# amathislab/myochallenge

Hardware: AMD Instinct MI355X
Metric: env-steps/sec (Baoding, 4096 envs) (higher is better)
Workload: dtype f64

## Files before the change

myochallenge_amd/csrc/myo_ppo_mlp.h:

```cpp
#pragma once
#ifndef MYO_EMU

typedef __attribute__((ext_vector_type(8))) __bf16 myo_bf16x8;
typedef __attribute__((ext_vector_type(4))) float myo_f32x4;

#define MLP_H 256
#define MLP_OPMAX 128
#define MLP_APM 48
#define MLP_AKP 64
#define MLP_XS (MLP_OPMAX + 8)
#define MLP_HS (MLP_H + 8)
#define MLP_DS (MLP_AKP + 8)
#define MLP_SOS 49
#define MLP_SPLITK 16

struct MlpArgs {
  const float *obs, *act, *oldlp, *adv, *ret;
  const long long* idx;
  const float *log_std, *adv_stats;
  const unsigned short *W1p, *W2, *W2T, *Whp, *WhT;
  const float* bias;
  unsigned short *XT, *H1T, *H2T, *dH1T, *dH2T, *dOT;
  float* part;
  int B, O, A, OP, NB;
// ... 79 lines not shown
  constexpr int PER = 4;
  float v[PER];
  float s = 0.f;
#pragma unroll
  for (int k = 0; k < PER; ++k) { const int i = lo + t + 256 * k; v[k] = i < hi ? adv[idx[i]] : 0.f; s += v[k]; }
  for (int i = lo + t + 256 * PER; i < hi; i += 256) s += adv[idx[i]];
  for (int off = 32; off >= 1; off >>= 1) s += __shfl_xor(s, off, 64);
  if ((t & 63) == 0) red[t >> 6] = s;
  __syncthreads();
  if (t == 0) s_mean = n ? ((red[0] + red[1]) + (red[2] + red[3])) / n : 0.f;
  __syncthreads();
  const float mean = s_mean;
  float m2 = 0.f;
#pragma unroll
  for (int k = 0; k < PER; ++k) { const float d = v[k] - mean; m2 += (lo + t + 256 * k) < hi ? d * d : 0.f; }
  for (int i = lo + t + 256 * PER; i < hi; i += 256) { const float d = adv[idx[i]] - mean; m2 += d * d; }
  for (int off = 32; off >= 1; off >>= 1) m2 += __shfl_xor(m2, off, 64);
  __syncthreads();
  if ((t & 63) == 0) red[t >> 6] = m2;
  __syncthreads();
  if (t == 0) { part[3 * blockIdx.x] = (float)n; part[3 * blockIdx.x + 1] = mean; part[3 * blockIdx.x + 2] = (red[0] + red[1]) + (red[2] + red[3]); }
}

template <int KSTEPS>
__device__ __forceinline__ void mlp_load_w(myo_bf16x8 (&bw)[8][4], const unsigned short* Wg, int w_stride, int n0, int lm, int lq) {
#pragma unroll
  for (int ks = 0; ks < KSTEPS; ++ks)
#pragma unroll
    for (int nt = 0; nt < 4; ++nt) bw[ks][nt] = *reinterpret_cast<const myo_bf16x8*>(Wg + (size_t)(n0 + 16 * nt + lm) * w_stride + 32 * ks + 8 * lq);
  __builtin_amdgcn_sched_barrier(0);
}
template <int KSTEPS, int MT>
__device__ __forceinline__ void mlp_mma_slab(myo_f32x4 (&acc)[MT][4], const unsigned short* As, int as_stride, const myo_bf16x8 (&bw)[8][4],
                                             int lm, int lq) {
#pragma unroll
  for (int mt = 0; mt < MT; ++mt)
#pragma unroll
    for (int nt = 0; nt < 4; ++nt) acc[mt][nt] = myo_f32x4{0.f, 0.f, 0.f, 0.f};
#pragma unroll
  for (int ks = 0; ks < KSTEPS; ++ks) {
#pragma unroll
    for (int m2 = 0; m2 < MT; m2 += 2) {
      myo_bf16x8 a[2];
#pragma unroll
      for (int mt = 0; mt < 2; ++mt) a[mt] = *reinterpret_cast<const myo_bf16x8*>(As + (16 * (m2 + mt) + lm) * as_stride + 32 * ks + 8 * lq);
#pragma unroll
      for (int mt = 0; mt < 2; ++mt)
#pragma unroll
        for (int nt = 0; nt < 4; ++nt) acc[m2 + mt][nt] = __builtin_amdgcn_mfma_f32_16x16x32_bf16(a[mt], bw[ks][nt], acc[m2 + mt][nt], 0, 0, 0);
    }
  }
  __builtin_amdgcn_sched_barrier(0);
}

#ifdef MLP_PROF
__device__ unsigned long long g_mlp_prof[16];
#define MLP_STAMP(k) { __syncthreads(); if (threadIdx.x == 0 && blockIdx.x == 3 && blockIdx.y == 0) g_mlp_prof[k] = wall_clock64(); }
extern "C" int myo_debug_mlp_prof(unsigned long long* out) { return (int)hipMemcpyFromSymbol(out, HIP_SYMBOL(g_mlp_prof), sizeof g_mlp_prof); }
#else
#define MLP_STAMP(k)
#endif

#ifndef MLP_BM
#define MLP_BM 32
#endif
#define MLP_FWDBWD_LDS (512 + MLP_BM * MLP_XS * 2 + MLP_BM * MLP_HS * 2 + MLP_BM * MLP_SOS * 4 + MLP_BM * MLP_DS * 2 + 128 * 4 + 192 * 4)

template <int MT>
__device__ __forceinline__ unsigned long long mlp_store_act(const myo_f32x4 (&acc)[MT][4], const float (&bb)[4], unsigned short* Hs, unsigned short* HT,
                                                            size_t B, int r0, int n0, int lm, int lq) {
  static_assert(MT * 16 <= 64, "one mask bit per accumulator element");
  unsigned long long mask = 0;
#pragma unroll
  for (int mt = 0; mt < MT; ++mt)
#pragma unroll
    for (int nt = 0; nt < 4; ++nt) {
      const int n = n0 + 16 * nt + lm, m = 16 * mt + 4 * lq;
      unsigned short h[4];
#pragma unroll
      for (int r = 0; r < 4; ++r) {
        h[r] = mlp_f2bf(fmaxf(acc[mt][nt][r] + bb[nt], 0.f)); Hs[(m + r) * MLP_HS + n] = h[r];
        mask |= (unsigned long long)(h[r] != 0) << (16 * mt + 4 * nt + r);
      }
      *reinterpret_cast<uint2*>(HT + (size_t)n * B + r0 + m) = make_uint2((unsigned)h[0] | ((unsigned)h[1] << 16), (unsigned)h[2] | ((unsigned)h[3] << 16));
    }
  return mask;
}
template <int MT, bool TO_LDS>
__device__ __forceinline__ void mlp_store_grad(const myo_f32x4 (&acc)[MT][4], unsigned long long mask, unsigned short* Hs, unsigned short* HT, size_t B,
                                               int r0, int n0, int lm, int lq) {
#pragma unroll
  for (int mt = 0; mt < MT; ++mt)
#pragma unroll
    for (int nt = 0; nt < 4; ++nt) {
      const int n = n0 + 16 * nt + lm, m = 16 * mt + 4 * lq;
      unsigned short h[4];
#pragma unroll
      for (int r = 0; r < 4; ++r) {
        const unsigned short on = (unsigned short)(-(int)((mask >> (16 * mt + 4 * nt + r)) & 1ull));
        h[r] = mlp_f2bf(acc[mt][nt][r]) & on;
        if (TO_LDS) Hs[(m + r) * MLP_HS + n] = h[r];
      }
      *reinterpret_cast<uint2*>(HT + (size_t)n * B + r0 + m) = make_uint2((unsigned)h[0] | ((unsigned)h[1] << 16), (unsigned)h[2] | ((unsigned)h[3] << 16));
    }
}

__global__ void __launch_bounds__(256, 2) k_mlp_fwdbwd(MlpArgs P) {
  constexpr int H = MLP_H, XS = MLP_XS, HS = MLP_HS, DS = MLP_DS, SOS = MLP_SOS, BM = MLP_BM, MT = BM / 16, RW = BM / 4;
  extern __shared__ __align__(16) unsigned char mlp_smem[];
  long long* s_idx = reinterpret_cast<long long*>(mlp_smem);
  unsigned short* Xs = reinterpret_cast<unsigned short*>(mlp_smem + 512);
  float* So = reinterpret_cast<float*>(mlp_smem + 512);
  unsigned short* Hs = Xs + BM * XS;
  float* Sa = reinterpret_cast<float*>(Hs + BM * HS);
  unsigned short* dOs = reinterpret_cast<unsigned short*>(Sa + BM * SOS);
  float* s_ls = reinterpret_cast<float*>(dOs + BM * DS);
  float* s_row = s_ls + 128;
  static_assert(BM * MLP_SOS * 4 <= BM * MLP_XS * 2, "the head output tile fits where X was");
  static_assert(BM == 32 || BM == 64, "wave / tile mapping below");
  const int t = threadIdx.x, w = t >> 6, lane = t & 63, lm = lane & 15, lq = lane >> 4;
  const int net = blockIdx.y, blk = blockIdx.x, r0 = blk * BM, B = P.B, O = P.O, A = P.A, OP = P.OP;
  const int n0 = 64 * w;
  MLP_STAMP(0)
  if (t < BM) s_idx[t] = P.idx[r0 + t];
  if (t < A) { const float ls = P.log_std[t]; s_ls[t] = ls; s_ls[64 + t] = __expf(-ls); }
  const float* b1 = P.bias + net * H; const float* b2 = P.bias + 2 * H + net * H; const float* bh = P.bias + 4 * H + net * MLP_APM;
  float bb1[4], bb2[4];
#pragma unroll
  for (int nt = 0; nt < 4; ++nt) { bb1[nt] = b1[n0 + 16 * nt + lm]; bb2[nt] = b2[n0 + 16 * nt + lm]; }
  myo_bf16x8 bw[8][4];
  {
    const unsigned short* W1 = P.W1p + (size_t)net * H * OP;
    if (OP == 96) mlp_load_w<3>(bw, W1, OP, n0, lm, lq);
    else if (OP == 128) mlp_load_w<4>(bw, W1, OP, n0, lm, lq);
    else if (OP == 64) mlp_load_w<2>(bw, W1, OP, n0, lm, lq);
    else mlp_load_w<1>(bw, W1, OP, n0, lm, lq);
  }
  __syncthreads();
  if (t < BM) {
    const size_t src = (size_t)s_idx[t];
    s_row[t] = P.adv[src]; s_row[64 + t] = P.oldlp[src]; s_row[128 + t] = P.ret[src];
  }
  {
    float v[RW][2], av[RW];
#pragma unroll
    for (int k = 0; k < RW; ++k) {
      const size_t row = (size_t)s_idx[RW * w + k];
      v[k][0] = lane < O ? P.obs[row * O + lane] : 0.f;
      v[k][1] = lane + 64 < O ? P.obs[row * O + lane + 64] : 0.f;
      av[k] = (net == 0 && lane < A) ? P.act[row * A + lane] : 0.f;
    }
#pragma unroll
    for (int k = 0; k < RW; ++k) {
      Xs[(RW * w + k) * XS + lane] = mlp_f2bf(v[k][0]);
      if (lane + 64 < OP) Xs[(RW * w + k) * XS + lane + 64] = mlp_f2bf(v[k][1]);
      if (lane < A) Sa[(RW * w + k) * SOS + lane] = av[k];
    }
    if (net == 0) {
#pragma unroll
      for (int h = 0; h < 2; ++h) {
        const int c = lane + 64 * h;
        if (c < OP) {
          unsigned u[RW / 2];
#pragma unroll
          for (int k = 0; k < RW / 2; ++k) u[k] = (unsigned)mlp_f2bf(v[2 * k][h]) | ((unsigned)mlp_f2bf(v[2 * k + 1][h]) << 16);
          uint4* dst = reinterpret_cast<uint4*>(P.XT + (size_t)c * B + r0 + RW * w);
#pragma unroll
          for (int q = 0; q < RW / 8; ++q) dst[q] = make_uint4(u[4 * q], u[4 * q + 1], u[4 * q + 2], u[4 * q + 3]);
        }
      }
    }
  }
  __syncthreads();
  MLP_STAMP(1)
  myo_f32x4 acc[MT][4];
  if (OP == 96) mlp_mma_slab<3, MT>(acc, Xs, XS, bw, lm, lq);
  else if (OP == 128) mlp_mma_slab<4, MT>(acc, Xs, XS, bw, lm, lq);
  else if (OP == 64) mlp_mma_slab<2, MT>(acc, Xs, XS, bw, lm, lq);
  else mlp_mma_slab<1, MT>(acc, Xs, XS, bw, lm, lq);
  mlp_load_w<H / 32>(bw, P.W2 + (size_t)net * H * H, H, n0, lm, lq);
  const unsigned long long mask1 = mlp_store_act<MT>(acc, bb1, Hs, P.H1T + (size_t)net * H * B, B, r0, n0, lm, lq);
  __syncthreads();
  MLP_STAMP(2)
  mlp_mma_slab<H / 32, MT>(acc, Hs, HS, bw, lm, lq);
  const unsigned short* Wh = P.Whp + (size_t)net * MLP_APM * H;
  myo_bf16x8 bh2[H / 32];
  if (w < 3) {
#pragma unroll
    for (int ks = 0; ks < H / 32; ++ks) bh2[ks] = *reinterpret_cast<const myo_bf16x8*>(Wh + (size_t)(16 * w + lm) * H + 32 * ks + 8 * lq);
  }
  __builtin_amdgcn_sched_barrier(0);
  __syncthreads();
  const unsigned long long mask2 = mlp_store_act<MT>(acc, bb2, Hs, P.H2T + (size_t)net * H * B, B, r0, n0, lm, lq);
  __syncthreads();
  MLP_STAMP(3)
  if (w < 3) {
    const float bv = bh[16 * w + lm];
#pragma unroll
    for (int mt = 0; mt < MT; ++mt) {
      myo_f32x4 ah = myo_f32x4{0.f, 0.f, 0.f, 0.f};
#pragma unroll
      for (int ks = 0; ks < H / 32; ++ks) {
        const myo_bf16x8 a = *reinterpret_cast<const myo_bf16x8*>(Hs + (16 * mt + lm) * HS + 32 * ks + 8 * lq);
        ah = __builtin_amdgcn_mfma_f32_16x16x32_bf16(a, bh2[ks], ah, 0, 0, 0);
      }
#pragma unroll
      for (int r = 0; r < 4; ++r) So[(16 * mt + 4 * lq + r) * SOS + 16 * w + lm] = ah[r] + bv;
    }
  }
  mlp_load_w<MLP_AKP / 32>(bw, P.WhT + (size_t)net * H * MLP_AKP, MLP_AKP, n0, lm, lq);
  __syncthreads();
  MLP_STAMP(4)
  const int NB = P.NB;
  if (w == 0) {
    const int r = lane < BM ? lane : 0;
    const bool on = lane < BM;
    if (net == 0) {
      float logp = 0.f;
      for (int a = 0; a < A; ++a) {
        const float z = (Sa[r * SOS + a] - So[r * SOS + a]) * s_ls[64 + a];
        logp += -0.5f * z * z - s_ls[a] - 0.9189385332046727f;
      }
      const float an = (s_row[r] - P.adv_stats[0]) / (P.adv_stats[1] + 1e-8f);
      const float clip = P.hp ? P.hp[MYO_HP_CLIP] : P.clip;
      const float lr_i = logp - s_row[64 + r];
      const float ratio = __expf(lr_i);
      const float s1 = an * ratio;
      const float rc = fminf(fmaxf(ratio, 1.f - clip), 1.f + clip);
      const float s2 = an * rc;
      float pl_i = on ? -fminf(s1, s2) / B : 0.f;
      const bool inside = (ratio > 1.f - clip) && (ratio < 1.f + clip);
      const float dlogp = -(an * ratio) * ((s1 <= s2) ? 1.f : (inside ? 1.f : 0.f)) / B;
      if (on) {
        for (int a = 0; a < A; ++a) {
          const float inv = s_ls[64 + a];
          const float z = (Sa[r * SOS + a] - So[r * SOS + a]) * inv;
          const float dm = dlogp * z * inv;
          So[r * SOS + a] = dm;
          Sa[r * SOS + a] = dlogp * (z * z - 1.f);
          dOs[r * DS + a] = mlp_f2bf(dm);
        }
        for (int a = A; a < MLP_AKP; ++a) dOs[r * DS + a] = 0;
      }
      for (int off = 32; off >= 1; off >>= 1) pl_i += __shfl_xor(pl_i, off, 64);
      if (lane == 0) P.part[(size_t)A * NB + blk] = pl_i;
      if (P.hp) {
        float ent = 0.f;
        for (int a = 0; a < A; ++a) ent += s_ls[a] + 1.4189385332046727f;
        float kl_i = on ? ((ratio - 1.f) - lr_i) / B : 0.f, cf_i = on ? (fabsf(ratio - 1.f) > clip ? 1.f : 0.f) / B : 0.f;
        float el_i = on ? -ent / B : 0.f;
        for (int off = 32; off >= 1; off >>= 1) {
          kl_i += __shfl_xor(kl_i, off, 64); cf_i += __shfl_xor(cf_i, off, 64); el_i += __shfl_xor(el_i, off, 64);
        }
        if (lane == 0) {
          P.part[(size_t)(2 * A + 3) * NB + blk] = kl_i; P.part[(size_t)(2 * A + 4) * NB + blk] = cf_i;
          P.part[(size_t)(2 * A + 5) * NB + blk] = el_i;
        }
      }
    } else {
      const float dv = So[r * SOS] - s_row[128 + r];
      float vl_i = on ? dv * dv / B : 0.f, dv_i = on ? P.vf_coef * 2.f / B * dv : 0.f;
      if (on) {
        dOs[r * DS] = mlp_f2bf(dv_i);
        for (int a = 1; a < MLP_AKP; ++a) dOs[r * DS + a] = 0;
      }
      for (int off = 32; off >= 1; off >>= 1) { vl_i += __shfl_xor(vl_i, off, 64); dv_i += __shfl_xor(dv_i, off, 64); }
      if (lane == 0) { P.part[(size_t)(A + 1) * NB + blk] = vl_i; P.part[(size_t)(2 * A + 2) * NB + blk] = dv_i; }
    }
  }
  __syncthreads();
  MLP_STAMP(5)
  if (net == 0 && t < A) {
    float my_ls = 0.f, my_db = 0.f;
    for (int r = 0; r < BM; ++r) { my_ls += Sa[r * SOS + t]; my_db += So[r * SOS + t]; }
    P.part[(size_t)t * NB + blk] = my_ls; P.part[(size_t)(A + 2 + t) * NB + blk] = my_db;
  }
  {
    const int Ah = net == 0 ? A : 1;
    for (int e = t; e < Ah * (BM / 8); e += 256) {
      const int c = e / (BM / 8), ch = e % (BM / 8);
      unsigned v[4];
#pragma unroll
      for (int k = 0; k < 4; ++k) v[k] = (unsigned)dOs[(8 * ch + 2 * k) * DS + c] | ((unsigned)dOs[(8 * ch + 2 * k + 1) * DS + c] << 16);
      *reinterpret_cast<uint4*>(P.dOT + ((size_t)net * 128 + c) * B + r0 + 8 * ch) = make_uint4(v[0], v[1], v[2], v[3]);
    }
  }
  MLP_STAMP(6)
  mlp_mma_slab<MLP_AKP / 32, MT>(acc, dOs, DS, bw, lm, lq);
  mlp_load_w<H / 32>(bw, P.W2T + (size_t)net * H * H, H, n0, lm, lq);
  mlp_store_grad<MT, true>(acc, mask2, Hs, P.dH2T + (size_t)net * H * B, B, r0, n0, lm, lq);
  __syncthreads();
  MLP_STAMP(7)
  mlp_mma_slab<H / 32, MT>(acc, Hs, HS, bw, lm, lq);
  mlp_store_grad<MT, false>(acc, mask1, Hs, P.dH1T + (size_t)net * H * B, B, r0, n0, lm, lq);
  MLP_STAMP(8)
}

struct MlpPolicyArgs {
  const float* obs;
  const float* log_std;
  const unsigned short *W1p, *W2, *Whp;
  const float* bias;
  float* obs_buf;
  float *act_buf, *val_buf, *logp_buf, *clipped;
  const int* t_idx;
  unsigned long long* draw_counter;
  unsigned long long seed;
  int N, O, A, OP, deterministic;
};
#define MLP_POLICY_LDS (MLP_BM * MLP_XS * 2 + MLP_BM * MLP_HS * 2 + 128 * 4)

template <int MT>
__device__ __forceinline__ void mlp_store_act_lds(const myo_f32x4 (&acc)[MT][4], const float (&bb)[4], unsigned short* Hs, int n0, int lm, int lq) {
#pragma unroll
  for (int mt = 0; mt < MT; ++mt)
#pragma unroll
    for (int nt = 0; nt < 4; ++nt) {
      const int n = n0 + 16 * nt + lm, m = 16 * mt + 4 * lq;
#pragma unroll
      for (int r = 0; r < 4; ++r) Hs[(m + r) * MLP_HS + n] = mlp_f2bf(fmaxf(acc[mt][nt][r] + bb[nt], 0.f));
    }
}

__global__ void __launch_bounds__(256, 2) k_mlp_policy(MlpPolicyArgs P) {
  constexpr int H = MLP_H, XS = MLP_XS, HS = MLP_HS, SOS = MLP_SOS, BM = MLP_BM, MT = BM / 16, RW = BM / 4;
  extern __shared__ __align__(16) unsigned char mlp_smem[];
  unsigned short* Xs = reinterpret_cast<unsigned short*>(mlp_smem);
  float* So = reinterpret_cast<float*>(mlp_smem);
  unsigned short* Hs = Xs + BM * XS;
  float* s_ls = reinterpret_cast<float*>(Hs + BM * HS);
  static_assert(BM * MLP_SOS * 4 <= BM * MLP_XS * 2, "the head output tile fits where X was");
  const int t = threadIdx.x, w = t >> 6, lane = t & 63, lm = lane & 15, lq = lane >> 4;
  const int net = blockIdx.y, r0 = blockIdx.x * BM, N = P.N, O = P.O, A = P.A, OP = P.OP;
  const int n0 = 64 * w;
  const size_t tt = (size_t)(*P.t_idx);
  if (t < A) { const float ls = P.log_std[t]; s_ls[t] = ls; s_ls[64 + t] = __expf(ls); }
  const float* b1 = P.bias + net * H; const float* b2 = P.bias + 2 * H + net * H; const float* bh = P.bias + 4 * H + net * MLP_APM;
  float bb1[4], bb2[4];
#pragma unroll
  for (int nt = 0; nt < 4; ++nt) { bb1[nt] = b1[n0 + 16 * nt + lm]; bb2[nt] = b2[n0 + 16 * nt + lm]; }
  myo_bf16x8 bw[8][4];
  {
    const unsigned short* W1 = P.W1p + (size_t)net * H * OP;
    if (OP == 96) mlp_load_w<3>(bw, W1, OP, n0, lm, lq);
    else if (OP == 128) mlp_load_w<4>(bw, W1, OP, n0, lm, lq);
    else if (OP == 64) mlp_load_w<2>(bw, W1, OP, n0, lm, lq);
    else mlp_load_w<1>(bw, W1, OP, n0, lm, lq);
  }
  {
    float v[RW][2];
#pragma unroll
    for (int k = 0; k < RW; ++k) {
      const size_t row = (size_t)(r0 + RW * w + k);
      v[k][0] = lane < O ? P.obs[row * O + lane] : 0.f;
      v[k][1] = lane + 64 < O ? P.obs[row * O + lane + 64] : 0.f;
    }
#pragma unroll
    for (int k = 0; k < RW; ++k) {
      Xs[(RW * w + k) * XS + lane] = mlp_f2bf(v[k][0]);
      if (lane + 64 < OP) Xs[(RW * w + k) * XS + lane + 64] = mlp_f2bf(v[k][1]);
      if (net == 0 && P.obs_buf) {
        float* dst = P.obs_buf + (tt * N + (size_t)(r0 + RW * w + k)) * O;
        if (lane < O) dst[lane] = v[k][0];
        if (lane + 64 < O) dst[lane + 64] = v[k][1];
      }
    }
  }
  __syncthreads();
  myo_f32x4 acc[MT][4];
  if (OP == 96) mlp_mma_slab<3, MT>(acc, Xs, XS, bw, lm, lq);
  else if (OP == 128) mlp_mma_slab<4, MT>(acc, Xs, XS, bw, lm, lq);
  else if (OP == 64) mlp_mma_slab<2, MT>(acc, Xs, XS, bw, lm, lq);
  else mlp_mma_slab<1, MT>(acc, Xs, XS, bw, lm, lq);
  mlp_load_w<H / 32>(bw, P.W2 + (size_t)net * H * H, H, n0, lm, lq);
  mlp_store_act_lds<MT>(acc, bb1, Hs, n0, lm, lq);
  __syncthreads();
  mlp_mma_slab<H / 32, MT>(acc, Hs, HS, bw, lm, lq);
  const unsigned short* Wh = P.Whp + (size_t)net * MLP_APM * H;
  myo_bf16x8 bh2[H / 32];
  if (w < 3) {
#pragma unroll
    for (int ks = 0; ks < H / 32; ++ks) bh2[ks] = *reinterpret_cast<const myo_bf16x8*>(Wh + (size_t)(16 * w + lm) * H + 32 * ks + 8 * lq);
  }
  __builtin_amdgcn_sched_barrier(0);
  __syncthreads();
  mlp_store_act_lds<MT>(acc, bb2, Hs, n0, lm, lq);
  __syncthreads();
  if (w < 3) {
    const float bv = bh[16 * w + lm];
#pragma unroll
    for (int mt = 0; mt < MT; ++mt) {
      myo_f32x4 ah = myo_f32x4{0.f, 0.f, 0.f, 0.f};
#pragma unroll
      for (int ks = 0; ks < H / 32; ++ks) {
        const myo_bf16x8 a = *reinterpret_cast<const myo_bf16x8*>(Hs + (16 * mt + lm) * HS + 32 * ks + 8 * lq);
        ah = __builtin_amdgcn_mfma_f32_16x16x32_bf16(a, bh2[ks], ah, 0, 0, 0);
      }
#pragma unroll
      for (int r = 0; r < 4; ++r) So[(16 * mt + 4 * lq + r) * SOS + 16 * w + lm] = ah[r] + bv;
    }
  }
  __syncthreads();
  if (net == 1) {
    if (t < BM) P.val_buf[tt * N + r0 + t] = So[t * SOS];
    return;
  }
  const unsigned long long ctr = P.draw_counter[0];
  const int row = t >> 3, g0 = t & 7, i = r0 + row;
  float logp = 0.f;
  static_assert(BM * 8 == 256, "8 lanes per row");
  for (int a0 = 4 * g0; a0 < A; a0 += 32) {
    unsigned int c[4] = {(unsigned int)i, (unsigned int)(a0 >> 2), (unsigned int)ctr, (unsigned int)(ctr >> 32)};
    unsigned int k0 = (unsigned int)P.seed, k1 = (unsigned int)(P.seed >> 32);
    for (int r = 0; r < 10; ++r) { philox_round(c, k0, k1); k0 += 0x9E3779B9u; k1 += 0xBB67AE85u; }
    float z[4];
    for (int h = 0; h < 2; ++h) {
      const float u1 = ((float)(c[2 * h] >> 8) + 0.5f) * (1.0f / 16777216.0f);
      const float u2 = ((float)(c[2 * h + 1] >> 8) + 0.5f) * (1.0f / 16777216.0f);
      const float rad = sqrtf(-2.0f * __logf(u1));
      float sn, cs;
      __sincosf(6.283185307179586f * u2, &sn, &cs);
      z[2 * h] = rad * cs; z[2 * h + 1] = rad * sn;
    }
#pragma unroll
    for (int k = 0; k < 4; ++k) {
      const int a = a0 + k;
      if (a < A) {
        const float mu = So[row * SOS + a], ls = s_ls[a];
        const float act = P.deterministic ? mu : mu + s_ls[64 + a] * z[k];
        const float zz = (act - mu) * __expf(-ls);
        logp += -0.5f * zz * zz - ls - 0.9189385332046727f;
        P.act_buf[(tt * N + i) * A + a] = act;
        P.clipped[(size_t)i * A + a] = fminf(fmaxf(act, -1.f), 1.f);
// ... 143 lines not shown
```

myochallenge_amd/csrc/myobatch.hip:

```cpp
#include <hip/hip_runtime.h>
#include <utility>
#include <vector>
#define MYO_BACKEND_NAME "gfx950"
#define MYO_BACKEND_DENSE_NEWTON 0
#define MYO_BACKEND_BATCH_FIELDS hipEvent_t ev0, ev1; std::vector<std::pair<hipEvent_t, hipEvent_t>> pending;
#include "myo_host.h"

typedef hipStream_t be_stream;
static int be_malloc(void** p, size_t n) { return (int)hipMalloc(p, n ? n : 1); }
static void be_free(void* p) { (void)hipFree(p); }
static int be_h2d(void* d, const void* h, size_t n) { return (int)hipMemcpy(d, h, n, hipMemcpyHostToDevice); }
static int be_set_device(int dev) { return (int)hipSetDevice(dev); }
static const char* be_errstr(int e) { return hipGetErrorString((hipError_t)e); }

#define MYO_MAX_DEVICES 64
struct BoundDev { const myo_batch* b = nullptr; hipStream_t last = nullptr; bool have_last = false; hipEvent_t ev = nullptr; };
static BoundDev g_bound[MYO_MAX_DEVICES];
static std::mutex g_bound_mu;
struct SlotWs { double* p = nullptr; int* map = nullptr; int users = 0; char* big = nullptr; int big_users = 0; };
static SlotWs g_slot_ws[MYO_MAX_DEVICES];
static bool slot_workspace_acquire(int device, double** ws, int** map) {
  if (device < 0 || device >= MYO_MAX_DEVICES) return false;
  std::lock_guard<std::mutex> lk(g_bound_mu);
  SlotWs& w = g_slot_ws[device];
// ... 1793 lines not shown
  hipStream_t st = (hipStream_t)stream;
  static bool lds_set = false;
  if (!lds_set) {
    if (hipFuncSetAttribute((const void*)k_mlp_fwdbwd, hipFuncAttributeMaxDynamicSharedMemorySize, MLP_FWDBWD_LDS) != hipSuccess)
      return fail(MYO_E_DEVICE, "myo_ppo_mlp_step: cannot reserve %d bytes of LDS", (int)MLP_FWDBWD_LDS);
    lds_set = true;
  }
  if (d->compute_adv_stats) hipLaunchKernelGGL(k_adv_moments, dim3(MLP_ADV_BLOCKS), dim3(256), 0, st, d->adv, (const long long*)d->idx, B, w.advpart);
  MlpPrepArgs pp;
  pp.p = d->params; pp.O = O; pp.OP = OP; pp.Ah[0] = A; pp.Ah[1] = 1;
  for (int k = 0; k < 2; ++k) {
    pp.off_W1[k] = d->off_W1[k]; pp.off_b1[k] = d->off_b1[k]; pp.off_W2[k] = d->off_W2[k]; pp.off_b2[k] = d->off_b2[k];
    pp.off_Wh[k] = d->off_Wh[k]; pp.off_bh[k] = d->off_bh[k];
  }
  pp.adv_part = w.advpart; pp.adv_stats = d->adv_stats; pp.adv_nb = d->compute_adv_stats ? MLP_ADV_BLOCKS : 0; pp.B = B;
  pp.W1p = w.W1p; pp.W2 = w.W2; pp.W2T = w.W2T; pp.Whp = w.Whp; pp.WhT = w.WhT; pp.bias = w.bias;
  hipLaunchKernelGGL(k_mlp_prep, dim3(256), dim3(256), 0, st, pp);
  MlpArgs a;
  a.obs = d->obs; a.act = d->act; a.oldlp = d->oldlp; a.adv = d->adv; a.ret = d->ret; a.idx = (const long long*)d->idx;
  a.log_std = d->params + d->off_log_std; a.adv_stats = d->adv_stats;
  a.W1p = w.W1p; a.W2 = w.W2; a.W2T = w.W2T; a.Whp = w.Whp; a.WhT = w.WhT; a.bias = w.bias;
  a.XT = w.XT; a.H1T = w.H1T; a.H2T = w.H2T; a.dH1T = w.dH1T; a.dH2T = w.dH2T; a.dOT = w.dOT; a.part = w.part;
  a.B = B; a.O = O; a.A = A; a.OP = OP; a.NB = B / MLP_BM; a.clip = d->clip; a.vf_coef = d->vf_coef; a.hp = d->hp;
  hipLaunchKernelGGL(k_mlp_fwdbwd, dim3(B / MLP_BM, 2), dim3(256), MLP_FWDBWD_LDS, st, a);
  MlpWgradArgs g;
  g.njobs = 0; g.B = B; g.rows_per_split = B / MLP_SPLITK; g.G = d->G; g.slab = w.slab;
  const size_t HB = (size_t)MLP_H * B;
  for (int net = 0; net < 2; ++net) {
    for (int m0 = 0; m0 < MLP_H; m0 += 128) {
      for (int n0 = 0; n0 < MLP_H; n0 += 128)
        g.job[g.njobs++] = MlpWgradJob{w.dH2T + net * HB, w.H1T + net * HB, MLP_H, MLP_H, MLP_H, m0, n0, d->off_W2[net], n0 == 0 ? d->off_b2[net] : -1};
      g.job[g.njobs++] = MlpWgradJob{w.dH1T + net * HB, w.XT, MLP_H, O, O, m0, 0, d->off_W1[net], d->off_b1[net]};
    }
    for (int n0 = 0; n0 < MLP_H; n0 += 128)
      g.job[g.njobs++] = MlpWgradJob{w.dOT + (size_t)net * 128 * B, w.H2T + net * HB, net == 0 ? A : 1, MLP_H, MLP_H, 0, n0, d->off_Wh[net], -1};
  }
  hipLaunchKernelGGL(k_mlp_wgrad, dim3(g.njobs * MLP_SPLITK), dim3(256), 0, st, g);
  if (d->sqnorm_part && d->adam_step) {
    MlpRfArgs rf;
    rf.slab = w.slab; rf.g = d->grads; rf.G = d->G; rf.splits = MLP_SPLITK; rf.part = w.part; rf.acc = d->acc; rf.NB = B / MLP_BM; rf.A = A;
    rf.ent_coef = d->ent_coef; rf.off_log_std = d->off_log_std; rf.off_bh0 = d->off_bh[0]; rf.off_bh1 = d->off_bh[1];
    rf.sq_part = d->sqnorm_part; rf.adam_step = d->adam_step; rf.hp = d->hp;
    hipLaunchKernelGGL(k_mlp_reduce_finish, dim3(MLP_RF_BLOCKS + 2 * A + 3), dim3(256), 0, st, rf);
  } else {
    hipLaunchKernelGGL(k_mlp_reduce, dim3((unsigned)((d->G + 255) / 256)), dim3(256), 0, st, (const float*)w.slab, d->grads, d->G, MLP_SPLITK);
    hipLaunchKernelGGL(k_colmajor_finish, dim3(2 * A + 3 + (d->hp ? 1 : 0)), dim3(64), 0, st, (const float*)w.part, d->acc, B / MLP_BM, A, d->ent_coef,
                       d->grads + d->off_log_std, d->grads + d->off_bh[0], d->grads + d->off_bh[1], d->hp);
// ... 31 lines not shown
  pp.p = d->params; pp.O = d->O; pp.OP = OP; pp.Ah[0] = d->A; pp.Ah[1] = 1;
  for (int k = 0; k < 2; ++k) {
    pp.off_W1[k] = d->off_W1[k]; pp.off_b1[k] = d->off_b1[k]; pp.off_W2[k] = d->off_W2[k]; pp.off_b2[k] = d->off_b2[k];
    pp.off_Wh[k] = d->off_Wh[k]; pp.off_bh[k] = d->off_bh[k];
  }
  pp.adv_part = nullptr; pp.adv_stats = nullptr; pp.adv_nb = 0; pp.B = 0;
  pp.W1p = w.W1p; pp.W2 = w.W2; pp.W2T = w.W2T; pp.Whp = w.Whp; pp.WhT = w.WhT; pp.bias = w.bias;
  hipLaunchKernelGGL(k_mlp_prep, dim3(256), dim3(256), 0, (hipStream_t)stream, pp);
  LAUNCH_CHECK(0)
  return MYO_OK;
}
extern "C" int myo_ppo_mlp_rollout(const myo_ppo_mlp_rollout_desc* d, void* stream) {
  if (!d || !d->obs || !d->params || !d->draw_counter || !d->t_idx || !d->act_buf || !d->val_buf || !d->logp_buf || !d->clipped || !d->workspace)
    return fail(MYO_E_ARG, "myo_ppo_mlp_rollout: null argument");
  if (!mlp_rollout_ok(d)) return fail(MYO_E_UNSUPPORTED, "myo_ppo_mlp_rollout: needs hidden = %d, obs <= %d, act <= %d, envs a multiple of %d", MLP_H, MLP_OPMAX, MLP_APM, MLP_BM);
  const int OP = (d->O + 31) / 32 * 32;
  const MlpImg w = mlp_carve_images((unsigned char*)d->workspace, OP);
  if ((long long)w.bytes > d->workspace_bytes) return fail(MYO_E_ARG, "myo_ppo_mlp_rollout: workspace too small (%zu bytes needed)", w.bytes);
  MlpPolicyArgs a;
  a.obs = d->obs; a.log_std = d->params + d->off_log_std; a.W1p = w.W1p; a.W2 = w.W2; a.Whp = w.Whp; a.bias = w.bias;
  a.obs_buf = d->obs_buf; a.act_buf = d->act_buf; a.val_buf = d->val_buf; a.logp_buf = d->logp_buf; a.clipped = d->clipped;
  a.t_idx = d->t_idx; a.draw_counter = (unsigned long long*)d->draw_counter; a.seed = d->seed;
  a.N = d->N; a.O = d->O; a.A = d->A; a.OP = OP; a.deterministic = d->deterministic;
  hipLaunchKernelGGL(k_mlp_policy, dim3(d->N / MLP_BM, 2), dim3(256), MLP_POLICY_LDS, (hipStream_t)stream, a);
  LAUNCH_CHECK(0)
  return MYO_OK;
}

#include "myo_lstm_step.h"
extern "C" int myo_lstm_step_supported(int H) { return (H == 32 || H == 64 || H == 128 || H == 256) ? 1 : 0; }
extern "C" int myo_lstm_step_fwd(const void* gx, long long gx_sg, long long gx_sr, const void* h_prev, const void* c_prev, const void* w_hh,
                                 const float* keep_next, int G, int N, int H, void* out_h, long long out_sg, void* hm_next, void* cm_next,
                                 void* c_new, void* ws, const float* c_prev32, float* cm_next32, void* stream) {
  if (!gx || !h_prev || (!c_prev && !c_prev32) || !w_hh || !out_h || !hm_next || (!cm_next && !cm_next32) || G <= 0 || N <= 0 || H <= 0 || (gx_sg & 3) || (gx_sr & 3) || (out_sg & 3))
    return fail(MYO_E_ARG, "myo_lstm_step_fwd: bad arguments");
  if (!myo_lstm_step_supported(H)) return fail(MYO_E_UNSUPPORTED, "myo_lstm_step_fwd: hidden size %d (32, 64, 128 or 256)", H);
  typedef const unsigned short* cu;
  typedef unsigned short* mu;
#define MYO_LSTM_FWD(HH)                                                                                                              \
  lstm_step_fwd_launch<HH>((cu)gx, gx_sg, gx_sr, (cu)h_prev, (cu)c_prev, (cu)w_hh, keep_next, G, N, (mu)out_h, out_sg, (mu)hm_next,   \
                           (mu)cm_next, (mu)c_new, (mu)ws, c_prev32, cm_next32, (hipStream_t)stream)
  switch (H) {
    case 32: MYO_LSTM_FWD(32); break;
    case 64: MYO_LSTM_FWD(64); break;
    case 128: MYO_LSTM_FWD(128); break;
    default: MYO_LSTM_FWD(256); break;
  }
// ... 61 lines not shown
```

Before: 1.727 million.

## Split MLP kernels across eight waves and parallelize the log-prob epilogue

Widens the fused PPO MLP forward/backward and policy kernels from 4 to 8 waves per block, so each wave owns 32 hidden columns instead of 64. This halves the per-wave weight-register and accumulator footprint and raises occupancy per block. The serial single-wave log-prob and gradient epilogue is redistributed so every wave handles its own rows, one action column per lane, with an extra LDS staging tile and additional barriers. The trade-off is more block-wide synchronisation, and in the policy kernel half the threads leave early during the sampling tail.

Result: no change. 1.739 million (median of 6 runs) (+0.7%).

```diff
diff --git a/myochallenge_amd/csrc/myo_ppo_mlp.h b/myochallenge_amd/csrc/myo_ppo_mlp.h
--- a/myochallenge_amd/csrc/myo_ppo_mlp.h
+++ b/myochallenge_amd/csrc/myo_ppo_mlp.h
@@ -125,21 +125,24 @@
   if (t == 0) { part[3 * blockIdx.x] = (float)n; part[3 * blockIdx.x + 1] = mean; part[3 * blockIdx.x + 2] = (red[0] + red[1]) + (red[2] + red[3]); }
 }
 
-template <int KSTEPS>
-__device__ __forceinline__ void mlp_load_w(myo_bf16x8 (&bw)[8][4], const unsigned short* Wg, int w_stride, int n0, int lm, int lq) {
+#define MLP_WAVES 8
+#define MLP_NT (MLP_H / 16 / MLP_WAVES)
+#define MLP_THREADS (64 * MLP_WAVES)
+template <int KSTEPS, int NT>
+__device__ __forceinline__ void mlp_load_w(myo_bf16x8 (&bw)[8][NT], const unsigned short* Wg, int w_stride, int n0, int lm, int lq) {
 #pragma unroll
   for (int ks = 0; ks < KSTEPS; ++ks)
 #pragma unroll
-    for (int nt = 0; nt < 4; ++nt) bw[ks][nt] = *reinterpret_cast<const myo_bf16x8*>(Wg + (size_t)(n0 + 16 * nt + lm) * w_stride + 32 * ks + 8 * lq);
+    for (int nt = 0; nt < NT; ++nt) bw[ks][nt] = *reinterpret_cast<const myo_bf16x8*>(Wg + (size_t)(n0 + 16 * nt + lm) * w_stride + 32 * ks + 8 * lq);
   __builtin_amdgcn_sched_barrier(0);
 }
-template <int KSTEPS, int MT>
-__device__ __forceinline__ void mlp_mma_slab(myo_f32x4 (&acc)[MT][4], const unsigned short* As, int as_stride, const myo_bf16x8 (&bw)[8][4],
+template <int KSTEPS, int MT, int NT>
+__device__ __forceinline__ void mlp_mma_slab(myo_f32x4 (&acc)[MT][NT], const unsigned short* As, int as_stride, const myo_bf16x8 (&bw)[8][NT],
                                              int lm, int lq) {
 #pragma unroll
   for (int mt = 0; mt < MT; ++mt)
 #pragma unroll
-    for (int nt = 0; nt < 4; ++nt) acc[mt][nt] = myo_f32x4{0.f, 0.f, 0.f, 0.f};
+    for (int nt = 0; nt < NT; ++nt) acc[mt][nt] = myo_f32x4{0.f, 0.f, 0.f, 0.f};
 #pragma unroll
   for (int ks = 0; ks < KSTEPS; ++ks) {
 #pragma unroll
@@ -150,7 +153,7 @@
 #pragma unroll
       for (int mt = 0; mt < 2; ++mt)
 #pragma unroll
-        for (int nt = 0; nt < 4; ++nt) acc[m2 + mt][nt] = __builtin_amdgcn_mfma_f32_16x16x32_bf16(a[mt], bw[ks][nt], acc[m2 + mt][nt], 0, 0, 0);
+        for (int nt = 0; nt < NT; ++nt) acc[m2 + mt][nt] = __builtin_amdgcn_mfma_f32_16x16x32_bf16(a[mt], bw[ks][nt], acc[m2 + mt][nt], 0, 0, 0);
     }
   }
   __builtin_amdgcn_sched_barrier(0);
@@ -169,38 +172,38 @@
 #endif
 #define MLP_FWDBWD_LDS (512 + MLP_BM * MLP_XS * 2 + MLP_BM * MLP_HS * 2 + MLP_BM * MLP_SOS * 4 + MLP_BM * MLP_DS * 2 + 128 * 4 + 192 * 4)
 
-template <int MT>
-__device__ __forceinline__ unsigned long long mlp_store_act(const myo_f32x4 (&acc)[MT][4], const float (&bb)[4], unsigned short* Hs, unsigned short* HT,
-                                                            size_t B, int r0, int n0, int lm, int lq) {
-  static_assert(MT * 16 <= 64, "one mask bit per accumulator element");
-  unsigned long long mask = 0;
+template <int MT, int NT>
+__device__ __forceinline__ unsigned mlp_store_act(const myo_f32x4 (&acc)[MT][NT], const float (&bb)[NT], unsigned short* Hs, unsigned short* HT,
+                                                  size_t B, int r0, int n0, int lm, int lq) {
+  static_assert(MT * NT * 4 <= 32, "one mask bit per accumulator element");
+  unsigned mask = 0;
 #pragma unroll
   for (int mt = 0; mt < MT; ++mt)
 #pragma unroll
-    for (int nt = 0; nt < 4; ++nt) {
+    for (int nt = 0; nt < NT; ++nt) {
       const int n = n0 + 16 * nt + lm, m = 16 * mt + 4 * lq;
       unsigned short h[4];
 #pragma unroll
       for (int r = 0; r < 4; ++r) {
         h[r] = mlp_f2bf(fmaxf(acc[mt][nt][r] + bb[nt], 0.f)); Hs[(m + r) * MLP_HS + n] = h[r];
-        mask |= (unsigned long long)(h[r] != 0) << (16 * mt + 4 * nt + r);
+        mask |= (unsigned)(h[r] != 0) << (4 * NT * mt + 4 * nt + r);
       }
       *reinterpret_cast<uint2*>(HT + (size_t)n * B + r0 + m) = make_uint2((unsigned)h[0] | ((unsigned)h[1] << 16), (unsigned)h[2] | ((unsigned)h[3] << 16));
     }
   return mask;
 }
-template <int MT, bool TO_LDS>
-__device__ __forceinline__ void mlp_store_grad(const myo_f32x4 (&acc)[MT][4], unsigned long long mask, unsigned short* Hs, unsigned short* HT, size_t B,
+template <int MT, int NT, bool TO_LDS>
+__device__ __forceinline__ void mlp_store_grad(const myo_f32x4 (&acc)[MT][NT], unsigned mask, unsigned short* Hs, unsigned short* HT, size_t B,
                                                int r0, int n0, int lm, int lq) {
 #pragma unroll
   for (int mt = 0; mt < MT; ++mt)
 #pragma unroll
-    for (int nt = 0; nt < 4; ++nt) {
+    for (int nt = 0; nt < NT; ++nt) {
       const int n = n0 + 16 * nt + lm, m = 16 * mt + 4 * lq;
       unsigned short h[4];
 #pragma unroll
       for (int r = 0; r < 4; ++r) {
-        const unsigned short on = (unsigned short)(-(int)((mask >> (16 * mt + 4 * nt + r)) & 1ull));
+        const unsigned short on = (unsigned short)(-(int)((mask >> (4 * NT * mt + 4 * nt + r)) & 1u));
         h[r] = mlp_f2bf(acc[mt][nt][r]) & on;
         if (TO_LDS) Hs[(m + r) * MLP_HS + n] = h[r];
       }
@@ -208,36 +211,39 @@
     }
 }
 
-__global__ void __launch_bounds__(256, 2) k_mlp_fwdbwd(MlpArgs P) {
-  constexpr int H = MLP_H, XS = MLP_XS, HS = MLP_HS, DS = MLP_DS, SOS = MLP_SOS, BM = MLP_BM, MT = BM / 16, RW = BM / 4;
+__global__ void __launch_bounds__(MLP_THREADS, 4) k_mlp_fwdbwd(MlpArgs P) {
+  constexpr int H = MLP_H, XS = MLP_XS, HS = MLP_HS, DS = MLP_DS, SOS = MLP_SOS, BM = MLP_BM, MT = BM / 16, NT = MLP_NT, NW = MLP_WAVES, RW = BM / NW;
   extern __shared__ __align__(16) unsigned char mlp_smem[];
   long long* s_idx = reinterpret_cast<long long*>(mlp_smem);
   unsigned short* Xs = reinterpret_cast<unsigned short*>(mlp_smem + 512);
   float* So = reinterpret_cast<float*>(mlp_smem + 512);
   unsigned short* Hs = Xs + BM * XS;
+  float* St = reinterpret_cast<float*>(Hs);
   float* Sa = reinterpret_cast<float*>(Hs + BM * HS);
   unsigned short* dOs = reinterpret_cast<unsigned short*>(Sa + BM * SOS);
   float* s_ls = reinterpret_cast<float*>(dOs + BM * DS);
   float* s_row = s_ls + 128;
   static_assert(BM * MLP_SOS * 4 <= BM * MLP_XS * 2, "the head output tile fits where X was");
+  static_assert(BM * MLP_SOS * 4 <= BM * MLP_HS * 2, "the log-prob terms fit where H2 was");
   static_assert(BM == 32 || BM == 64, "wave / tile mapping below");
+  static_assert(NT * 16 * NW == H && (RW == 4 || RW == 8), "wave / column mapping below");
   const int t = threadIdx.x, w = t >> 6, lane = t & 63, lm = lane & 15, lq = lane >> 4;
   const int net = blockIdx.y, blk = blockIdx.x, r0 = blk * BM, B = P.B, O = P.O, A = P.A, OP = P.OP;
-  const int n0 = 64 * w;
+  const int n0 = 16 * NT * w;
   MLP_STAMP(0)
   if (t < BM) s_idx[t] = P.idx[r0 + t];
   if (t < A) { const float ls = P.log_std[t]; s_ls[t] = ls; s_ls[64 + t] = __expf(-ls); }
   const float* b1 = P.bias + net * H; const float* b2 = P.bias + 2 * H + net * H; const float* bh = P.bias + 4 * H + net * MLP_APM;
-  float bb1[4], bb2[4];
-#pragma unroll
-  for (int nt = 0; nt < 4; ++nt) { bb1[nt] = b1[n0 + 16 * nt + lm]; bb2[nt] = b2[n0 + 16 * nt + lm]; }
-  myo_bf16x8 bw[8][4];
+  float bb1[NT], bb2[NT];
+#pragma unroll
+  for (int nt = 0; nt < NT; ++nt) { bb1[nt] = b1[n0 + 16 * nt + lm]; bb2[nt] = b2[n0 + 16 * nt + lm]; }
+  myo_bf16x8 bw[8][NT];
   {
     const unsigned short* W1 = P.W1p + (size_t)net * H * OP;
-    if (OP == 96) mlp_load_w<3>(bw, W1, OP, n0, lm, lq);
-    else if (OP == 128) mlp_load_w<4>(bw, W1, OP, n0, lm, lq);
-    else if (OP == 64) mlp_load_w<2>(bw, W1, OP, n0, lm, lq);
-    else mlp_load_w<1>(bw, W1, OP, n0, lm, lq);
+    if (OP == 96) mlp_load_w<3, NT>(bw, W1, OP, n0, lm, lq);
+    else if (OP == 128) mlp_load_w<4, NT>(bw, W1, OP, n0, lm, lq);
+    else if (OP == 64) mlp_load_w<2, NT>(bw, W1, OP, n0, lm, lq);
+    else mlp_load_w<1, NT>(bw, W1, OP, n0, lm, lq);
   }
   __syncthreads();
   if (t < BM) {
@@ -267,25 +273,25 @@
           unsigned u[RW / 2];
 #pragma unroll
           for (int k = 0; k < RW / 2; ++k) u[k] = (unsigned)mlp_f2bf(v[2 * k][h]) | ((unsigned)mlp_f2bf(v[2 * k + 1][h]) << 16);
-          uint4* dst = reinterpret_cast<uint4*>(P.XT + (size_t)c * B + r0 + RW * w);
-#pragma unroll
-          for (int q = 0; q < RW / 8; ++q) dst[q] = make_uint4(u[4 * q], u[4 * q + 1], u[4 * q + 2], u[4 * q + 3]);
+          uint2* dst = reinterpret_cast<uint2*>(P.XT + (size_t)c * B + r0 + RW * w);
+#pragma unroll
+          for (int q = 0; q < RW / 4; ++q) dst[q] = make_uint2(u[2 * q], u[2 * q + 1]);
         }
       }
     }
   }
   __syncthreads();
   MLP_STAMP(1)
-  myo_f32x4 acc[MT][4];
-  if (OP == 96) mlp_mma_slab<3, MT>(acc, Xs, XS, bw, lm, lq);
-  else if (OP == 128) mlp_mma_slab<4, MT>(acc, Xs, XS, bw, lm, lq);
-  else if (OP == 64) mlp_mma_slab<2, MT>(acc, Xs, XS, bw, lm, lq);
-  else mlp_mma_slab<1, MT>(acc, Xs, XS, bw, lm, lq);
-  mlp_load_w<H / 32>(bw, P.W2 + (size_t)net * H * H, H, n0, lm, lq);
-  const unsigned long long mask1 = mlp_store_act<MT>(acc, bb1, Hs, P.H1T + (size_t)net * H * B, B, r0, n0, lm, lq);
+  myo_f32x4 acc[MT][NT];
+  if (OP == 96) mlp_mma_slab<3, MT, NT>(acc, Xs, XS, bw, lm, lq);
+  else if (OP == 128) mlp_mma_slab<4, MT, NT>(acc, Xs, XS, bw, lm, lq);
+  else if (OP == 64) mlp_mma_slab<2, MT, NT>(acc, Xs, XS, bw, lm, lq);
+  else mlp_mma_slab<1, MT, NT>(acc, Xs, XS, bw, lm, lq);
+  mlp_load_w<H / 32, NT>(bw, P.W2 + (size_t)net * H * H, H, n0, lm, lq);
+  const unsigned mask1 = mlp_store_act<MT, NT>(acc, bb1, Hs, P.H1T + (size_t)net * H * B, B, r0, n0, lm, lq);
   __syncthreads();
   MLP_STAMP(2)
-  mlp_mma_slab<H / 32, MT>(acc, Hs, HS, bw, lm, lq);
+  mlp_mma_slab<H / 32, MT, NT>(acc, Hs, HS, bw, lm, lq);
   const unsigned short* Wh = P.Whp + (size_t)net * MLP_APM * H;
   myo_bf16x8 bh2[H / 32];
   if (w < 3) {
@@ -294,7 +300,7 @@
   }
   __builtin_amdgcn_sched_barrier(0);
   __syncthreads();
-  const unsigned long long mask2 = mlp_store_act<MT>(acc, bb2, Hs, P.H2T + (size_t)net * H * B, B, r0, n0, lm, lq);
+  const unsigned mask2 = mlp_store_act<MT, NT>(acc, bb2, Hs, P.H2T + (size_t)net * H * B, B, r0, n0, lm, lq);
   __syncthreads();
   MLP_STAMP(3)
   if (w < 3) {
@@ -311,19 +317,26 @@
       for (int r = 0; r < 4; ++r) So[(16 * mt + 4 * lq + r) * SOS + 16 * w + lm] = ah[r] + bv;
     }
   }
-  mlp_load_w<MLP_AKP / 32>(bw, P.WhT + (size_t)net * H * MLP_AKP, MLP_AKP, n0, lm, lq);
+  mlp_load_w<MLP_AKP / 32, NT>(bw, P.WhT + (size_t)net * H * MLP_AKP, MLP_AKP, n0, lm, lq);
   __syncthreads();
   MLP_STAMP(4)
   const int NB = P.NB;
-  if (w == 0) {
-    const int r = lane < BM ? lane : 0;
-    const bool on = lane < BM;
-    if (net == 0) {
+  if (net == 0) {
+    if (lane < A) {
+      const float inv = s_ls[64 + lane], ls = s_ls[lane];
+#pragma unroll
+      for (int k = 0; k < RW; ++k) {
+        const int r = RW * w + k;
+        const float z = (Sa[r * SOS + lane] - So[r * SOS + lane]) * inv;
+        St[r * SOS + lane] = -0.5f * z * z - ls - 0.9189385332046727f;
+      }
+    }
+    __syncthreads();
+    if (w == 0) {
+      const int r = lane < BM ? lane : 0;
+      const bool on = lane < BM;
       float logp = 0.f;
-      for (int a = 0; a < A; ++a) {
-        const float z = (Sa[r * SOS + a] - So[r * SOS + a]) * s_ls[64 + a];
-        logp += -0.5f * z * z - s_ls[a] - 0.9189385332046727f;
-      }
+      for (int a = 0; a < A; ++a) logp += St[r * SOS + a];
       const float an = (s_row[r] - P.adv_stats[0]) / (P.adv_stats[1] + 1e-8f);
       const float clip = P.hp ? P.hp[MYO_HP_CLIP] : P.clip;
       const float lr_i = logp - s_row[64 + r];
@@ -334,17 +347,7 @@
       float pl_i = on ? -fminf(s1, s2) / B : 0.f;
       const bool inside = (ratio > 1.f - clip) && (ratio < 1.f + clip);
       const float dlogp = -(an * ratio) * ((s1 <= s2) ? 1.f : (inside ? 1.f : 0.f)) / B;
-      if (on) {
-        for (int a = 0; a < A; ++a) {
-          const float inv = s_ls[64 + a];
-          const float z = (Sa[r * SOS + a] - So[r * SOS + a]) * inv;
-          const float dm = dlogp * z * inv;
-          So[r * SOS + a] = dm;
-          Sa[r * SOS + a] = dlogp * (z * z - 1.f);
-          dOs[r * DS + a] = mlp_f2bf(dm);
-        }
-        for (int a = A; a < MLP_AKP; ++a) dOs[r * DS + a] = 0;
-      }
+      if (on) s_row[128 + r] = dlogp;
       for (int off = 32; off >= 1; off >>= 1) pl_i += __shfl_xor(pl_i, off, 64);
       if (lane == 0) P.part[(size_t)A * NB + blk] = pl_i;
       if (P.hp) {
@@ -360,27 +363,51 @@
           P.part[(size_t)(2 * A + 5) * NB + blk] = el_i;
         }
       }
-    } else {
+    }
+    __syncthreads();
+#pragma unroll
+    for (int k = 0; k < RW; ++k) {
+      const int r = RW * w + k;
+      if (lane < A) {
+        const float inv = s_ls[64 + lane], dlogp = s_row[128 + r];
+        const float z = (Sa[r * SOS + lane] - So[r * SOS + lane]) * inv;
+        const float dm = dlogp * z * inv;
+        So[r * SOS + lane] = dm;
+        Sa[r * SOS + lane] = dlogp * (z * z - 1.f);
+        dOs[r * DS + lane] = mlp_f2bf(dm);
+      } else {
+        dOs[r * DS + lane] = 0;
+      }
+    }
+  } else {
+    if (w == 0) {
+      const int r = lane < BM ? lane : 0;
+      const bool on = lane < BM;
       const float dv = So[r * SOS] - s_row[128 + r];
       float vl_i = on ? dv * dv / B : 0.f, dv_i = on ? P.vf_coef * 2.f / B * dv : 0.f;
-      if (on) {
-        dOs[r * DS] = mlp_f2bf(dv_i);
-        for (int a = 1; a < MLP_AKP; ++a) dOs[r * DS + a] = 0;
-      }
+      if (on) s_row[r] = dv_i;
       for (int off = 32; off >= 1; off >>= 1) { vl_i += __shfl_xor(vl_i, off, 64); dv_i += __shfl_xor(dv_i, off, 64); }
       if (lane == 0) { P.part[(size_t)(A + 1) * NB + blk] = vl_i; P.part[(size_t)(2 * A + 2) * NB + blk] = dv_i; }
     }
-  }
+    __syncthreads();
+#pragma unroll
+    for (int k = 0; k < RW; ++k) {
+      const int r = RW * w + k;
+      dOs[r * DS + lane] = lane == 0 ? mlp_f2bf(s_row[r]) : (unsigned short)0;
+    }
+  }
+  static_assert(MLP_AKP == 64, "the d(head output) image is one column per lane");
   __syncthreads();
   MLP_STAMP(5)
-  if (net == 0 && t < A) {
-    float my_ls = 0.f, my_db = 0.f;
-    for (int r = 0; r < BM; ++r) { my_ls += Sa[r * SOS + t]; my_db += So[r * SOS + t]; }
-    P.part[(size_t)t * NB + blk] = my_ls; P.part[(size_t)(A + 2 + t) * NB + blk] = my_db;
+  if (net == 0 && w < 2 && lane < A) {
+    const float* S = w == 0 ? Sa : So;
+    float my = 0.f;
+    for (int r = 0; r < BM; ++r) my += S[r * SOS + lane];
+    P.part[(size_t)(w == 0 ? lane : A + 2 + lane) * NB + blk] = my;
   }
   {
     const int Ah = net == 0 ? A : 1;
-    for (int e = t; e < Ah * (BM / 8); e += 256) {
+    for (int e = t; e < Ah * (BM / 8); e += MLP_THREADS) {
       const int c = e / (BM / 8), ch = e % (BM / 8);
       unsigned v[4];
 #pragma unroll
@@ -389,13 +416,13 @@
     }
   }
   MLP_STAMP(6)
-  mlp_mma_slab<MLP_AKP / 32, MT>(acc, dOs, DS, bw, lm, lq);
-  mlp_load_w<H / 32>(bw, P.W2T + (size_t)net * H * H, H, n0, lm, lq);
-  mlp_store_grad<MT, true>(acc, mask2, Hs, P.dH2T + (size_t)net * H * B, B, r0, n0, lm, lq);
+  mlp_mma_slab<MLP_AKP / 32, MT, NT>(acc, dOs, DS, bw, lm, lq);
+  mlp_load_w<H / 32, NT>(bw, P.W2T + (size_t)net * H * H, H, n0, lm, lq);
+  mlp_store_grad<MT, NT, true>(acc, mask2, Hs, P.dH2T + (size_t)net * H * B, B, r0, n0, lm, lq);
   __syncthreads();
   MLP_STAMP(7)
-  mlp_mma_slab<H / 32, MT>(acc, Hs, HS, bw, lm, lq);
-  mlp_store_grad<MT, false>(acc, mask1, Hs, P.dH1T + (size_t)net * H * B, B, r0, n0, lm, lq);
+  mlp_mma_slab<H / 32, MT, NT>(acc, Hs, HS, bw, lm, lq);
+  mlp_store_grad<MT, NT, false>(acc, mask1, Hs, P.dH1T + (size_t)net * H * B, B, r0, n0, lm, lq);
   MLP_STAMP(8)
 }
 
@@ -413,20 +440,20 @@
 };
 #define MLP_POLICY_LDS (MLP_BM * MLP_XS * 2 + MLP_BM * MLP_HS * 2 + 128 * 4)
 
-template <int MT>
-__device__ __forceinline__ void mlp_store_act_lds(const myo_f32x4 (&acc)[MT][4], const float (&bb)[4], unsigned short* Hs, int n0, int lm, int lq) {
+template <int MT, int NT>
+__device__ __forceinline__ void mlp_store_act_lds(const myo_f32x4 (&acc)[MT][NT], const float (&bb)[NT], unsigned short* Hs, int n0, int lm, int lq) {
 #pragma unroll
   for (int mt = 0; mt < MT; ++mt)
 #pragma unroll
-    for (int nt = 0; nt < 4; ++nt) {
+    for (int nt = 0; nt < NT; ++nt) {
       const int n = n0 + 16 * nt + lm, m = 16 * mt + 4 * lq;
 #pragma unroll
       for (int r = 0; r < 4; ++r) Hs[(m + r) * MLP_HS + n] = mlp_f2bf(fmaxf(acc[mt][nt][r] + bb[nt], 0.f));
     }
 }
 
-__global__ void __launch_bounds__(256, 2) k_mlp_policy(MlpPolicyArgs P) {
-  constexpr int H = MLP_H, XS = MLP_XS, HS = MLP_HS, SOS = MLP_SOS, BM = MLP_BM, MT = BM / 16, RW = BM / 4;
+__global__ void __launch_bounds__(MLP_THREADS, 4) k_mlp_policy(MlpPolicyArgs P) {
+  constexpr int H = MLP_H, XS = MLP_XS, HS = MLP_HS, SOS = MLP_SOS, BM = MLP_BM, MT = BM / 16, NT = MLP_NT, RW = BM / MLP_WAVES;
   extern __shared__ __align__(16) unsigned char mlp_smem[];
   unsigned short* Xs = reinterpret_cast<unsigned short*>(mlp_smem);
   float* So = reinterpret_cast<float*>(mlp_smem);
@@ -435,20 +462,20 @@
   static_assert(BM * MLP_SOS * 4 <= BM * MLP_XS * 2, "the head output tile fits where X was");
   const int t = threadIdx.x, w = t >> 6, lane = t & 63, lm = lane & 15, lq = lane >> 4;
   const int net = blockIdx.y, r0 = blockIdx.x * BM, N = P.N, O = P.O, A = P.A, OP = P.OP;
-  const int n0 = 64 * w;
+  const int n0 = 16 * NT * w;
   const size_t tt = (size_t)(*P.t_idx);
   if (t < A) { const float ls = P.log_std[t]; s_ls[t] = ls; s_ls[64 + t] = __expf(ls); }
   const float* b1 = P.bias + net * H; const float* b2 = P.bias + 2 * H + net * H; const float* bh = P.bias + 4 * H + net * MLP_APM;
-  float bb1[4], bb2[4];
-#pragma unroll
-  for (int nt = 0; nt < 4; ++nt) { bb1[nt] = b1[n0 + 16 * nt + lm]; bb2[nt] = b2[n0 + 16 * nt + lm]; }
-  myo_bf16x8 bw[8][4];
+  float bb1[NT], bb2[NT];
+#pragma unroll
+  for (int nt = 0; nt < NT; ++nt) { bb1[nt] = b1[n0 + 16 * nt + lm]; bb2[nt] = b2[n0 + 16 * nt + lm]; }
+  myo_bf16x8 bw[8][NT];
   {
     const unsigned short* W1 = P.W1p + (size_t)net * H * OP;
-    if (OP == 96) mlp_load_w<3>(bw, W1, OP, n0, lm, lq);
-    else if (OP == 128) mlp_load_w<4>(bw, W1, OP, n0, lm, lq);
-    else if (OP == 64) mlp_load_w<2>(bw, W1, OP, n0, lm, lq);
-    else mlp_load_w<1>(bw, W1, OP, n0, lm, lq);
+    if (OP == 96) mlp_load_w<3, NT>(bw, W1, OP, n0, lm, lq);
+    else if (OP == 128) mlp_load_w<4, NT>(bw, W1, OP, n0, lm, lq);
+    else if (OP == 64) mlp_load_w<2, NT>(bw, W1, OP, n0, lm, lq);
+    else mlp_load_w<1, NT>(bw, W1, OP, n0, lm, lq);
   }
   {
     float v[RW][2];
@@ -470,15 +497,15 @@
     }
   }
   __syncthreads();
-  myo_f32x4 acc[MT][4];
-  if (OP == 96) mlp_mma_slab<3, MT>(acc, Xs, XS, bw, lm, lq);
-  else if (OP == 128) mlp_mma_slab<4, MT>(acc, Xs, XS, bw, lm, lq);
-  else if (OP == 64) mlp_mma_slab<2, MT>(acc, Xs, XS, bw, lm, lq);
-  else mlp_mma_slab<1, MT>(acc, Xs, XS, bw, lm, lq);
-  mlp_load_w<H / 32>(bw, P.W2 + (size_t)net * H * H, H, n0, lm, lq);
-  mlp_store_act_lds<MT>(acc, bb1, Hs, n0, lm, lq);
-  __syncthreads();
-  mlp_mma_slab<H / 32, MT>(acc, Hs, HS, bw, lm, lq);
+  myo_f32x4 acc[MT][NT];
+  if (OP == 96) mlp_mma_slab<3, MT, NT>(acc, Xs, XS, bw, lm, lq);
+  else if (OP == 128) mlp_mma_slab<4, MT, NT>(acc, Xs, XS, bw, lm, lq);
+  else if (OP == 64) mlp_mma_slab<2, MT, NT>(acc, Xs, XS, bw, lm, lq);
+  else mlp_mma_slab<1, MT, NT>(acc, Xs, XS, bw, lm, lq);
+  mlp_load_w<H / 32, NT>(bw, P.W2 + (size_t)net * H * H, H, n0, lm, lq);
+  mlp_store_act_lds<MT, NT>(acc, bb1, Hs, n0, lm, lq);
+  __syncthreads();
+  mlp_mma_slab<H / 32, MT, NT>(acc, Hs, HS, bw, lm, lq);
   const unsigned short* Wh = P.Whp + (size_t)net * MLP_APM * H;
   myo_bf16x8 bh2[H / 32];
   if (w < 3) {
@@ -487,7 +514,7 @@
   }
   __builtin_amdgcn_sched_barrier(0);
   __syncthreads();
-  mlp_store_act_lds<MT>(acc, bb2, Hs, n0, lm, lq);
+  mlp_store_act_lds<MT, NT>(acc, bb2, Hs, n0, lm, lq);
   __syncthreads();
   if (w < 3) {
     const float bv = bh[16 * w + lm];
@@ -508,10 +535,11 @@
     if (t < BM) P.val_buf[tt * N + r0 + t] = So[t * SOS];
     return;
   }
+  if (t >= BM * 8) return;
   const unsigned long long ctr = P.draw_counter[0];
   const int row = t >> 3, g0 = t & 7, i = r0 + row;
   float logp = 0.f;
-  static_assert(BM * 8 == 256, "8 lanes per row");
+  static_assert(BM * 8 <= MLP_THREADS, "8 lanes per row");
   for (int a0 = 4 * g0; a0 < A; a0 += 32) {
     unsigned int c[4] = {(unsigned int)i, (unsigned int)(a0 >> 2), (unsigned int)ctr, (unsigned int)(ctr >> 32)};
     unsigned int k0 = (unsigned int)P.seed, k1 = (unsigned int)(P.seed >> 32);
diff --git a/myochallenge_amd/csrc/myobatch.hip b/myochallenge_amd/csrc/myobatch.hip
--- a/myochallenge_amd/csrc/myobatch.hip
+++ b/myochallenge_amd/csrc/myobatch.hip
@@ -1839,7 +1839,7 @@
   a.W1p = w.W1p; a.W2 = w.W2; a.W2T = w.W2T; a.Whp = w.Whp; a.WhT = w.WhT; a.bias = w.bias;
   a.XT = w.XT; a.H1T = w.H1T; a.H2T = w.H2T; a.dH1T = w.dH1T; a.dH2T = w.dH2T; a.dOT = w.dOT; a.part = w.part;
   a.B = B; a.O = O; a.A = A; a.OP = OP; a.NB = B / MLP_BM; a.clip = d->clip; a.vf_coef = d->vf_coef; a.hp = d->hp;
-  hipLaunchKernelGGL(k_mlp_fwdbwd, dim3(B / MLP_BM, 2), dim3(256), MLP_FWDBWD_LDS, st, a);
+  hipLaunchKernelGGL(k_mlp_fwdbwd, dim3(B / MLP_BM, 2), dim3(MLP_THREADS), MLP_FWDBWD_LDS, st, a);
   MlpWgradArgs g;
   g.njobs = 0; g.B = B; g.rows_per_split = B / MLP_SPLITK; g.G = d->G; g.slab = w.slab;
   const size_t HB = (size_t)MLP_H * B;
@@ -1917,7 +1917,7 @@
   a.obs_buf = d->obs_buf; a.act_buf = d->act_buf; a.val_buf = d->val_buf; a.logp_buf = d->logp_buf; a.clipped = d->clipped;
   a.t_idx = d->t_idx; a.draw_counter = (unsigned long long*)d->draw_counter; a.seed = d->seed;
   a.N = d->N; a.O = d->O; a.A = d->A; a.OP = OP; a.deterministic = d->deterministic;
-  hipLaunchKernelGGL(k_mlp_policy, dim3(d->N / MLP_BM, 2), dim3(256), MLP_POLICY_LDS, (hipStream_t)stream, a);
+  hipLaunchKernelGGL(k_mlp_policy, dim3(d->N / MLP_BM, 2), dim3(MLP_THREADS), MLP_POLICY_LDS, (hipStream_t)stream, a);
   LAUNCH_CHECK(0)
   return MYO_OK;
 }
```
